# magicat777/Audio-Analyzer-OMEGA

Measured on AMD Instinct MI355X. Metric: audio frames/sec (multi-res FFT + LUFS + TruePeak) at 1/2/4/8 MI355X, higher is better.
Workload: dtype f32; 1 GPU; cfg2: 256 stereo frames x 16384 samples per GPU; MRFFT 16k/8k/4k/1k + combine(512) + K-weighted LUFS + 4x true peak + meter aggregates; channel_frames_per_gpu=512, frame_samples=16384, target_bins=512, parallelism=frames sharded over 1 GPU(s)

## Files before the change

audio-analyzer-omega_amd/csrc/capi.cpp:

```cpp
#include <hip/hip_runtime.h>

#include <algorithm>
#include <cmath>
#include <cstdarg>
#include <cstdio>
#include <cstdlib>
#include <cstring>
#include <exception>
#include <map>
#include <new>
#include <string>
#include <vector>

#include "../../include/omega.h"
#include "params.hpp"

namespace omega {
hipError_t launch_spectral(int W, const SpectralParams& p, hipStream_t s);
hipError_t launch_mrfft(const SpectralParams& p, hipStream_t s);
hipError_t launch_mrfft_range(const SpectralParams& p, int r0, int r1, hipStream_t s);
hipError_t launch_mrfft_independent(const SpectralParams& p, hipStream_t s);
hipError_t launch_truepeak(int W, const SpectralParams& p, hipStream_t s);
hipError_t launch_truepeak_rf(int W, const SpectralParams& p, hipStream_t s, int extra_lds = 0);
hipError_t launch_mrfft_rf(int n, const SpectralParams& p, int r, hipStream_t s);
// ... 167 lines not shown
  std::memcpy(P, An, sizeof P);
  double Pk[4] = {P[0], P[1], P[2], P[3]};
  for (int l = 0; l < 64; ++l) {
    for (int q = 0; q < 4; ++q) t.pw[l][q] = (float)Pk[q];
    mat2_mul(P, Pk, Pk);
  }
  return t;
}

}

struct omega_bands {
  omega_ctx* ctx;
  int op, n_bands, n_out, n_bins, n_valid;
  int32_t* d_starts;
  int32_t* d_ends;
  float* d_scale;
  float* d_bin_scale;
};

struct omega_ctx {
  omega_config cfg{};
  int device = 0;
  hipStream_t own = nullptr, stream = nullptr;
  hipStream_t cap = nullptr, fork[1] = {nullptr};
  std::vector<hipStream_t> spare;
  unsigned* d_probe = nullptr;
  unsigned probe_seq = 0;
  std::vector<hipStream_t> checked;
  bool queue_shared = false;
  hipEvent_t ev_fork = nullptr, ev_join[2] = {nullptr, nullptr};
  bool use_graph = false;
  int layout = 3;
  unsigned* d_kw_done = nullptr;
  unsigned kw_issued = 0;
  unsigned q_issued = 0;
  unsigned tp_issued = 0;
  unsigned prep_issued = 0;
  unsigned seg_issued = 0;
  unsigned lt_issued = 0;
  unsigned* tp_count_to = nullptr;
  bool side_meters = false;
  unsigned seg_par[2] = {0, 0};
  bool pipe = false;
  bool pend = false;
  MeterPrepParams pend_mq{};
  int pend_nq = 0, pend_par = 0;
  int stage_par = 0;
  unsigned* d_tail = nullptr;
  unsigned tail_issued = 0;
  unsigned long long* d_mirror = nullptr;
  unsigned mirror_gen = 0;
  int tail_ok = 0;
  unsigned* h_err = nullptr;
  unsigned* d_err = nullptr;
  int poll_limit = 1 << 22;
  float* d_lufs_scr = nullptr;
  int64_t lufs_scr_cap = 0;
  bool res_independent = false;
  hipEvent_t ev_kw = nullptr;
  struct GraphEntry {
    std::vector<uint64_t> key;
    hipGraph_t graph;
    hipGraphExec_t exec;
  };
  std::vector<GraphEntry> graphs;
  char err[512] = {};
  float2* d_tw[kMaxLog2] = {};

  float2* d_rot = nullptr;
  float* d_win[kMaxRes] = {};
  float* d_wgt[kMaxRes] = {};
  CombEnt* d_ent = nullptr;
  int ent_begin[kMaxRes] = {}, ent_end[kMaxRes] = {};
  int pair_lo[kMaxRes] = {}, pair_hi[kMaxRes] = {};
  int ent_jmax[kMaxRes] = {};
  std::map<std::pair<int, int>, BiquadTab*> kw_tabs;
  int rf_sizes = 1 << 14;
  std::map<std::pair<int, int>, float*> windows;
  std::map<int, float2*> rots;
  std::map<std::pair<int, int>, float4*> wgens;
  int* d_own_off = nullptr;
  int* d_own_rj = nullptr;
  float* d_own_frac = nullptr;
  std::map<int, std::pair<double*, std::pair<int, int>>> chroma_mats;
  double chroma_df = 0.0;
  struct ChromaTab {
    int n_bins = 0, lo = 0, hi = 0;
    double df = 0.0;
    float4* w4 = nullptr;
    float* w1 = nullptr;
    unsigned short* perm = nullptr;
    int* goff = nullptr;
    float* rec = nullptr;
  } ctab;
  int n_cu = 0;
  int drum_bins = 0, drum_cur = 0;
  float* d_dprev[2] = {};
  float* d_dhist[2] = {};
  int* d_dlen[2] = {};
  long long* d_dpos[2] = {};
  float* d_dflux = nullptr;
  PostParams post{};
  float* d_post_raw = nullptr;
  int64_t post_raw_cap = 0;
  double* d_vu_hist[2] = {};
// ... 58 lines not shown
  std::vector<void*> allocs;
};

namespace {

int fail(omega_ctx* c, int code, const char* fmt, ...) {
  char buf[512];
  va_list ap;
  va_start(ap, fmt);
  std::vsnprintf(buf, sizeof buf, fmt, ap);
  va_end(ap);
  if (c) {
    std::memcpy(c->err, buf, sizeof buf);
    c->zc_ok = false;
  }
  return code;
}

#define HIPC(ctx, x)                                                                           \
  do {                                                                                         \
    hipError_t e_ = (x);                                                                       \
    if (e_ != hipSuccess) return fail(ctx, OMEGA_EHIP, "%s: %s", #x, hipGetErrorString(e_)); \
  } while (0)

int guard_fail(omega_ctx* c) noexcept {
  try {
    throw;
  } catch (const std::bad_alloc&) {
    return fail(c, OMEGA_ENOMEM, "out of host memory");
  } catch (const std::exception& e) {
    return fail(c, OMEGA_EHIP, "internal error: %s", e.what());
  } catch (...) {
    return fail(c, OMEGA_EHIP, "internal error: unknown exception");
  }
}

template <class T>
int dalloc(omega_ctx* c, T** p, size_t count) {
  void* q = nullptr;
  const hipError_t e = hipMalloc(&q, std::max<size_t>(count, 1) * sizeof(T));
  if (e != hipSuccess) return fail(c, OMEGA_ENOMEM, "hipMalloc(%zu): %s", count * sizeof(T), hipGetErrorString(e));
  c->allocs.push_back(q);
  *p = static_cast<T*>(q);
  return 0;
}

template <class T>
int grow(omega_ctx* c, T** p, int64_t* cap, int64_t need) {
  if (need <= *cap) return 0;
  if (*p) {
    HIPC(c, hipStreamSynchronize(c->stream));
    for (hipStream_t f : c->fork)
      if (f) HIPC(c, hipStreamSynchronize(f));
    auto it = std::find(c->allocs.begin(), c->allocs.end(), static_cast<void*>(*p));
    if (it != c->allocs.end()) c->allocs.erase(it);
    (void)hipFree(*p);
    *p = nullptr;
    *cap = 0;
  }
  if (int e = dalloc(c, p, (size_t)need)) return e;
  *cap = need;
  return 0;
}

template <class T>
int upload(omega_ctx* c, T** p, const std::vector<T>& v) {
  int r = dalloc(c, p, v.size());
  if (r) return r;
  HIPC(c, hipMemcpy(*p, v.data(), v.size() * sizeof(T), hipMemcpyHostToDevice));
  return 0;
}

int stage_buf(omega_ctx* c, int i, size_t bytes, void** out) {
  if ((int)c->stage.size() <= i) c->stage.resize(i + 1);
  DevBuf& b = c->stage[i];
  if (b.n < bytes) {
    if (b.p) (void)hipFree(b.p);
    b.p = nullptr;
    b.n = 0;
    const hipError_t e = hipMalloc(&b.p, std::max<size_t>(bytes, 256));
    if (e != hipSuccess) return fail(c, OMEGA_ENOMEM, "staging hipMalloc(%zu): %s", bytes, hipGetErrorString(e));
    b.n = std::max<size_t>(bytes, 256);
  }
  *out = b.p;
  return 0;
}

int build_twiddles(omega_ctx* c) {
  for (int l = 1; l < kMaxLog2; ++l) {
    const int N = 1 << l;
    std::vector<float2> t(N);
    for (int m = 0; m < N; ++m) {
      const double a = 2.0 * kPi * (double)m / (double)N;
      t[m] = make_float2((float)std::cos(a), (float)-std::sin(a));
    }
    int r = upload(c, &c->d_tw[l], t);
    if (r) return r;
  }
  return 0;
}

int get_kw_tab(omega_ctx* c, int M, int L, BiquadTab** out) {
  const auto key = std::make_pair(M, L);
  auto it = c->kw_tabs.find(key);
  if (it != c->kw_tabs.end()) {
    *out = it->second;
    return 0;
  }
  const double fs = c->cfg.sample_rate;
  std::vector<BiquadTab> t = {make_biquad_tab(butter2_highpass(38.0, fs), L),
                              make_biquad_tab(butter2_highpass(1500.0, fs), L)};
  BiquadTab* d = nullptr;
  int r = upload(c, &d, t);
  if (r) return r;
  c->kw_tabs[key] = d;
  *out = d;
  return 0;
}
int get_kw_tab(omega_ctx* c, int M, BiquadTab** out) { return get_kw_tab(c, M, kw_chunk(M), out); }

int get_window(omega_ctx* c, int m, int kind, float** out) {
  auto key = std::make_pair(m, kind);
  auto it = c->windows.find(key);
  if (it != c->windows.end()) {
    *out = it->second;
    return 0;
  }
  float* d = nullptr;
  int r = upload(c, &d, make_window(m, kind));
  if (r) return r;
// ... 451 lines not shown
    p.n_t_in = c->d_nt[a];
    p.skeys_in = c->d_skeys[a];
    p.n_s_in = c->d_ns[a];
    p.t0_in = c->d_t0[a];
    p.hist_l_out = c->d_hist_l[b];
    p.hist_t_out = c->d_hist_t[b];
    p.n_l_out = c->d_nl[b];
    p.n_t_out = c->d_nt[b];
    p.skeys_out = c->d_skeys[b];
    p.n_s_out = c->d_ns[b];
    p.t0_out = c->d_t0[b];
    p.HL = c->HL;
    p.HT = c->HT;
    p.mom_len = c->cfg.momentary_len;
    p.short_len = c->cfg.short_len;
    p.int_len = c->cfg.integrated_len;
    p.peak_len = c->cfg.peak_len;
    p.poll_limit = c->poll_limit;
    p.err_word = c->d_err;
    p.gate = (float)c->cfg.gate_lufs;
    p.core = c->d_core[a];
    p.ext = c->d_ext[a];
    p.n_core = c->d_ncore[a];
    p.n_ext = c->d_next[a];
    p.gcount = c->d_gcount[a];
    p.gsum = c->d_gsum[a];
    p.out = out + f0 * C * OMEGA_N_METERS;
    p.parts = 3;
    p.seg_ctr = c->d_kw_done + 4;
    p.seg_pre_target = c->seg_par[a];
    p.seg_post_target = c->seg_par[b];
    v.push_back(p);
    c->cur = b;
  }
  return v;
}

int meters_enqueue(omega_ctx* c, const float* lufs, const float* tp, int64_t n_frames, double* out,
                   hipStream_t stream, hipEvent_t tp_ready, unsigned* wait_ctr = nullptr, unsigned wait_target = 0) {
  bool first = true;
  for (MeterPrepParams p : meter_chunks(c, lufs, tp, n_frames, out)) {
    if (first && wait_ctr) {
      p.wait_ctr = wait_ctr;
      p.wait_target = wait_target;
    }
    HIPC(c, launch_meter_prep(p, stream));
    if (tp_ready && first) HIPC(c, hipStreamWaitEvent(stream, tp_ready, 0));
    HIPC(c, launch_meter_query(p, stream));
    first = false;
  }
  return 0;
}

int flush_meters(omega_ctx* c) {
  if (!c->pend) return 0;
  HIPC(c, hipSetDevice(c->device));
  BatchPlan bp{};
  bp.q_begin = 0;
  bp.q_n = c->pend_nq;
  bp.seg_start[0] = bp.seg_start[1] = bp.multi_start = c->pend_nq;
  SpectralParams sp{};
  KWeightParams kp{};
  const hipError_t le = launch_batch(sp, kp, bp, c->pend_mq, c->pend_nq, c->stream);
  if (le != hipSuccess) return fail(c, OMEGA_EHIP, "meter segment launch: %s", hipGetErrorString(le));
  c->pend = false;
  c->seg_par[c->pend_par] = c->seg_issued + (unsigned)c->pend_nq;
  c->seg_issued += (unsigned)c->pend_nq;
  return 0;
}

bool batch_eligible(omega_ctx* c, const SpectralParams& sp, const KWeightParams& kp, int W, bool do_res, hipStream_t s,
                    int* mr) {
  *mr = -1;
  if (W != 16384 || (c->cap && s == c->cap)) return false;
  if ((kp.lufs_out || kp.weighted_out) && kp.mode != 0) return false;
  if (!do_res) return true;
  if (!c->res_independent) return false;
  for (int r = 0; r < sp.n_res; ++r) {
    if (!sp.comb_out && !sp.res[r].mag_out) continue;
    const int n = sp.res[r].n;
    if (n == 16384) {
      if (*mr >= 0 || !((sp.rf_sizes >> 14) & 1)) return false;
      *mr = r;
    } else if (n < 512 || n > 8192) {
      return false;
    }
  }
  return true;
}

int enqueue_batch(omega_ctx* c, SpectralParams sp, KWeightParams kp, int W, int64_t n_frames, const float* lufs,
                  const float* tp, double* meters, hipStream_t s, int mr, bool do_tp, bool do_kw, bool fold) {
  (void)W;
  const int64_t n = sp.n_cf;
  BatchPlan bp{};
  int seg[2][3], ns[2] = {0, 0};
  auto add = [&](int sg, int role, bool on) {
    if (on) seg[sg][ns[sg]++] = role;
  };
  add(0, 0, do_kw);
  add(0, 2, mr >= 0);
  add(1, 1, do_tp);
  const int64_t groups = (n + 7) / 8;
  int64_t end = 0;
  for (int sg = 0; sg < 2; ++sg) {
    bp.n_roles[sg] = ns[sg] ? ns[sg] : 1;
    for (int i = 0; i < 3; ++i) bp.roles[sg][i] = i < ns[sg] ? seg[sg][i] : 0;
    end += ns[sg] ? 8 * ns[sg] * groups : 0;
    if (end > 0x7FFFFFFF) return fail(c, OMEGA_EINVAL, "batch of %lld channel-frames too large", (long long)n);
    bp.seg_begin[sg + 1] = (int)end;
  }
  bp.mr_res = mr < 0 ? 0 : mr;
  int64_t nwg = 0;
  for (int r = 0; r < sp.n_res; ++r) {
    if (r == mr || (!sp.comb_out && !sp.res[r].mag_out)) continue;
    const int K = sp.res[r].n / 2;
    const int G = K / 16 < 64 ? 64 : K / 16;
    const int fpw = 512 / G;
    bp.multi.res[bp.multi.n_seg] = r;
    bp.multi.wg_begin[bp.multi.n_seg] = (int)nwg;
    ++bp.multi.n_seg;
    nwg += (n + fpw - 1) / fpw;
  }
  const bool in_grid = meters && do_tp && do_kw && n_frames > 0 && n_frames <= kChunkFrames;
  const int64_t n_mq = in_grid ? std::min<int64_t>((n + kBatchWaves - 1) / kBatchWaves, kMeterWgs) : 0;
  fold = fold && in_grid;
  const int64_t q_n = fold ? (c->pend ? c->pend_nq : 0) : n_mq;
  bp.pat = 1;
  bp.multi_n = (int)nwg;
  bp.seg_start[0] = 0;
  bp.seg_start[1] = bp.seg_begin[1];
  bp.multi_start = bp.seg_begin[2];
  const int64_t body_end = end + nwg;
  bp.q_begin = (int)body_end;
  bp.q_n = (int)q_n;
  if (fold) bp.q_begin = bp.multi_start;
  const int64_t grid = body_end + q_n;
  if (grid > 0x7FFFFFFF) return fail(c, OMEGA_EINVAL, "batch of %lld channel-frames too large", (long long)n);
  MeterPrepParams mq{};
  std::vector<MeterPrepParams> mc;
  if (in_grid) {
    const int a = c->cur;
    const unsigned seg_par_was = c->seg_par[a ^ 1];
    if (fold && c->pend) c->seg_par[c->pend_par] = c->seg_issued + (unsigned)c->pend_nq;
    const int cur_was = c->cur;
    mc = meter_chunks(c, lufs, tp, n_frames, meters);
    MeterPrepParams p = mc[0];
    p.q_done = c->d_kw_done + 3;
    const size_t mir_n = (size_t)kChunkFrames * c->cfg.n_channels;
    if (fold && !c->d_mirror) {
      HIPC(c, hipMalloc(&c->d_mirror, 2 * mir_n * sizeof(unsigned long long)));
      HIPC(c, hipMemset(c->d_mirror, 0, 2 * mir_n * sizeof(unsigned long long)));
    }
    const bool mirror = fold;
    const unsigned gen_was = c->mirror_gen;
    if (mirror) {
      c->mirror_gen = c->mirror_gen == 0xFFFFFFFFu ? 2u : c->mirror_gen + 1;
      kp.lufs_mirror = c->d_mirror + (c->mirror_gen & 1) * mir_n;
      kp.mirror_gen = c->mirror_gen;
      p.lufs_mirror = kp.lufs_mirror;
      p.mirror_gen = c->mirror_gen;
    } else {
      kp.kw_done = c->d_kw_done;
      c->kw_issued += (unsigned)n;
      p.wait_ctr = c->d_kw_done;
      p.wait_target = c->kw_issued;
    }
    if (fold && c->tail_ok == 0) {
      int ok = 0;
      HIPC(c, hipDeviceGetAttribute(&ok, hipDeviceAttributeCanUseStreamWaitValue, c->device));
      c->tail_ok = -1;
      if (ok && hipExtMallocWithFlags(reinterpret_cast<void**>(&c->d_tail), 8, hipMallocSignalMemory) == hipSuccess) {
        HIPC(c, hipMemset(c->d_tail, 0, 8));
        c->tail_issued = 0;
        c->tail_ok = 1;
      }
    }
    const bool tail = fold && c->tail_ok > 0;
    if (tail) bp.tail_ctr = c->d_tail;
    if (!fold) HIPC(c, launch_meter_prep(p, c->fork[0]));
    c->side_meters = true;
    mq = mc[0];
    mq.start_ctr = c->d_kw_done + 3;
    mq.start_target = c->prep_issued + (unsigned)p.C;
    if (!fold) {
      sp.tp_done = c->d_kw_done + 2;
      mq.join_ctr = c->d_kw_done + 2;
      mq.join_target = c->tp_issued + (unsigned)n;
    }
    const hipError_t le = launch_batch(sp, kp, bp, fold ? c->pend_mq : mq, (int)grid, s);
    if (le != hipSuccess) {
      if (!fold) {
        (void)hipMemcpy(c->d_kw_done, &c->kw_issued, sizeof(unsigned), hipMemcpyHostToDevice);
        c->prep_issued += (unsigned)p.C;
      } else {
        c->mirror_gen = gen_was;
        c->seg_par[a ^ 1] = seg_par_was;
        c->cur = cur_was;
      }
      return fail(c, OMEGA_EHIP, "batch launch: %s", hipGetErrorString(le));
    }
    if (!fold) c->tp_issued += (unsigned)n;
    if (tail) {
      HIPC(c, hipStreamWaitValue32(c->fork[0], c->d_tail, c->tail_issued + 1, hipStreamWaitValueGte, 0xFFFFFFFFu));
      ++c->tail_issued;
    }
    if (fold) HIPC(c, launch_meter_prep(p, c->fork[0]));
    c->side_meters = true;
    c->prep_issued += (unsigned)p.C;
    if (fold) {
      if (c->pend) c->seg_issued += (unsigned)c->pend_nq;
      c->pend = true;
      c->pend_mq = mq;
      c->pend_nq = (int)n_mq;
      c->pend_par = a;
    } else {
      c->seg_par[a] = c->seg_issued + (unsigned)n_mq;
      c->seg_issued += (unsigned)n_mq;
    }
    return 0;
  }
  if (meters) {
    mc = meter_chunks(c, lufs, tp, n_frames, meters);
    kp.kw_done = c->d_kw_done;
    c->kw_issued += (unsigned)n;
    for (size_t i = 0; i < mc.size(); ++i) {
      MeterPrepParams p = mc[i];
      if (i == 0) {
        p.wait_ctr = c->d_kw_done;
        p.wait_target = c->kw_issued;
      }
      HIPC(c, launch_meter_prep(p, c->fork[0]));
      c->side_meters = true;
      p.parts = 1;
      p.q_done = c->d_kw_done + 1;
      HIPC(c, launch_meter_query(p, c->fork[0]));
      c->side_meters = true;
      c->q_issued += (unsigned)(((p.n_frames + 3) / 4) * p.C);
    }
  }
  if (grid > 0) {
    const hipError_t le = launch_batch(sp, kp, bp, mq, (int)grid, s);
    if (le != hipSuccess) {
      if (meters) (void)hipMemcpy(c->d_kw_done, &c->kw_issued, sizeof(unsigned), hipMemcpyHostToDevice);
      return fail(c, OMEGA_EHIP, "batch launch: %s", hipGetErrorString(le));
    }
  }
  for (size_t i = 0; i < mc.size(); ++i) {
    MeterPrepParams p = mc[i];
    p.parts = 2;
    if (i + 1 == mc.size()) {
      p.join_ctr = c->d_kw_done + 1;
      p.join_target = c->q_issued;
    }
    HIPC(c, launch_meter_query(p, s));
  }
  return 0;
}

hipError_t create_side_stream(hipStream_t* st) { return hipStreamCreateWithFlags(st, hipStreamNonBlocking); }

constexpr int kProbePolls = 2048;
constexpr size_t kMaxSpare = 6;
int side_stream_check(omega_ctx* c, bool force = false) {
  if (!force && std::find(c->checked.begin(), c->checked.end(), c->stream) != c->checked.end()) return 0;
  if (!c->d_probe) {
    HIPC(c, hipMalloc(&c->d_probe, 2 * sizeof(unsigned)));
    HIPC(c, hipMemset(c->d_probe, 0, 2 * sizeof(unsigned)));
  }
  HIPC(c, hipStreamSynchronize(c->stream));
  HIPC(c, hipStreamSynchronize(c->fork[0]));
  for (int attempt = 0; attempt < 3; ++attempt) {
    const unsigned target = ++c->probe_seq;
    HIPC(c, launch_queue_probe(c->d_probe, target, kProbePolls, c->fork[0], c->stream));
    HIPC(c, hipStreamSynchronize(c->fork[0]));
    HIPC(c, hipStreamSynchronize(c->stream));
    unsigned r[2] = {0u, 0u};
    HIPC(c, hipMemcpy(r, c->d_probe, sizeof r, hipMemcpyDeviceToHost));
    if (r[1] == target) {
      c->queue_shared = false;
      c->checked.push_back(c->stream);
      return 0;
    }
    c->checked.clear();
    if (c->spare.size() >= kMaxSpare) {
      HIPC(c, hipStreamDestroy(c->spare.front()));
      c->spare.erase(c->spare.begin());
    }
    c->spare.push_back(c->fork[0]);
    c->fork[0] = nullptr;
    HIPC(c, create_side_stream(&c->fork[0]));
  }
  c->queue_shared = true;
  std::snprintf(c->err, sizeof c->err,
                "side stream: no hardware queue independent of the context's stream found after 3 attempts "
                "(more streams than GPU_MAX_HW_QUEUES?): batch-path device waits may run to their bound "
                "(OMEGA_POLL_LIMIT) and return OMEGA_EHIP");
  return 0;
}

int enqueue_frames(omega_ctx* c, SpectralParams sp, KWeightParams kp, int W, int64_t n_frames, const float* lufs,
                   const float* tp, double* meters, hipStream_t s, bool pipe = false, float* lufs_st = nullptr,
                   float* tp_st = nullptr) {
  const bool do_tp = sp.tp_out != nullptr, do_kw = kp.lufs_out || kp.weighted_out;
  const bool do_res = sp.comb_out != nullptr || sp.res[0].mag_out || sp.res[1].mag_out || sp.res[2].mag_out ||
                      sp.res[3].mag_out;
  int mr = -1;
  const bool batch = c->layout == 3 && batch_eligible(c, sp, kp, W, do_res, s, &mr);
  const bool fold = pipe && batch && meters && do_tp && do_kw && n_frames > 0 && n_frames <= kChunkFrames;
  if (c->pend && !fold)
    if (int e = flush_meters(c)) return e;
  if (fold && lufs_st && tp_st) {
    if (kp.lufs_out != lufs_st) kp.lufs_copy = kp.lufs_out;
    if (sp.tp_out != tp_st) sp.tp_copy = sp.tp_out;
    kp.lufs_out = lufs_st;
    sp.tp_out = tp_st;
    lufs = lufs_st;
    tp = tp_st;
  }
  if (batch) return enqueue_batch(c, sp, kp, W, n_frames, lufs, tp, meters, s, mr, do_tp, do_kw, fold);
  if (do_kw) HIPC(c, launch_kweight(W, kp, s));
  std::vector<MeterPrepParams> mc;
  if (meters) {
    mc = meter_chunks(c, lufs, tp, n_frames, meters);
    HIPC(c, hipEventRecord(c->ev_kw, s));
    HIPC(c, hipStreamWaitEvent(c->fork[0], c->ev_kw, 0));
    for (MeterPrepParams p : mc) {
      HIPC(c, launch_meter_prep(p, c->fork[0]));
      c->side_meters = true;
      p.parts = 1;
      HIPC(c, launch_meter_query(p, c->fork[0]));
      c->side_meters = true;
    }
    HIPC(c, hipEventRecord(c->ev_join[0], c->fork[0]));
  }
  if (do_res) HIPC(c, c->res_independent ? launch_mrfft_independent(sp, s) : launch_mrfft(sp, s));
  if (do_tp) HIPC(c, tp_launch(c, W, sp, s));
  for (MeterPrepParams p : mc) {
    p.parts = 2;
    HIPC(c, launch_meter_query(p, s));
  }
  if (meters) HIPC(c, hipStreamWaitEvent(s, c->ev_join[0], 0));
  return 0;
}

}

extern "C" {

const char* omega_version(void) { return "omega-mi355x 0.5 (gfx950, ABI 5)"; }

#ifdef OMEGA_STAMPS
int omega_dev_probe(omega_ctx* c, int which, const float* x, int64_t n_frames, float* comb, float* aux) {
  SpectralParams sp = spectral_params(c);
  const int W = c->cfg.frame_size;
  sp.x = x;
  sp.frame_stride = (int64_t)c->cfg.n_channels * W;
  sp.chan_stride = W;
  sp.n_cf = n_frames * c->cfg.n_channels;
  sp.comb_out = comb;
  (void)aux;
  for (int r = 0; r < kMaxRes; ++r) sp.res[r].mag_out = nullptr;
  hipError_t e = hipErrorInvalidValue;
  sp.tp_out = aux;
  float2* rot = nullptr;
  if (int r = get_rot(c, W, &rot)) return r;
  sp.rot = rot;
  if (which == 0) e = launch_mrfft_rf(16384, sp, 0, c->stream);
  if (which == 2) e = launch_truepeak_rf(16384, sp, c->stream);
  if (which == 3) e = launch_truepeak_rf(16384, sp, c->stream, 16 * 1024);
  return e == hipSuccess ? 0 : fail(c, OMEGA_EHIP, "probe %d: %s", which, hipGetErrorString(e));
// ... 902 lines not shown

int omega_post_reset(omega_ctx* c) try {
  if (!c) return OMEGA_EINVAL;
  if (!c->post.T) return 0;
  HIPC(c, hipSetDevice(c->device));
  HIPC(c, hipMemsetAsync(std::min(c->post.has_prev, c->post.has_prev_out), 0, 4 * sizeof(int), c->stream));
  HIPC(c, hipStreamSynchronize(c->stream));
  return 0;
} catch (...) {
  return guard_fail(c);
}

int omega_post_process(omega_ctx* c, const float* spectra, int64_t n_frames, int64_t stride, int32_t flags,
                       float bass_boost, float* spectrum_out, double* bands_out, int32_t* content_out) try {
  if (!c) return OMEGA_EINVAL;
  if (!c->post.T) return fail(c, OMEGA_EINVAL, "post process: omega_post_configure first");
  if (n_frames < 0 || stride < c->post.T || !spectra || !spectrum_out || (c->post.nb && !bands_out) ||
      n_frames > 0x7FFFFFFF)
    return fail(c, OMEGA_EINVAL, "post process: bad layout (n %lld, stride %lld, %d bins)", (long long)n_frames,
                (long long)stride, c->post.T);
  if (n_frames == 0) return 0;
  HIPC(c, hipSetDevice(c->device));
  PostParams p = c->post;
  p.in = spectra;
  p.n = n_frames;
  p.stride = stride;
  p.flags = flags;
  p.bass_boost = bass_boost;
  p.spec_out = spectrum_out;
  p.band_out = bands_out;
  p.content_out = content_out;
  const int64_t rows = n_frames + kEmaSpareRows, nch = (n_frames + 63) / 64;
  const int64_t pre_off = (rows * (c->post.nb + 1) + 1) / 2 * 2;
  if (c->post.nb) {
    if (int e = grow(c, &c->d_post_raw, &c->post_raw_cap, pre_off + 4 * nch * c->post.nb + 4)) return e;
  }
  p.band_raw = c->d_post_raw;
  p.frame64 = reinterpret_cast<int*>(c->d_post_raw + rows * c->post.nb);
  p.ema_pre = reinterpret_cast<double*>(c->d_post_raw + pre_off);
  p.ema_end = p.ema_pre + nch * c->post.nb;
  HIPC(c, launch_post(p, c->stream));
  if (c->post.nb) {
    std::swap(c->post.prev, c->post.prev_out);
    std::swap(c->post.has_prev, c->post.has_prev_out);
  }
  return 0;
} catch (...) {
  return guard_fail(c);
}

void omega_destroy(omega_ctx* c) try {
  if (!c) return;
  if (c->device >= 0) (void)hipSetDevice(c->device);
  if (c->pend && !flush_meters(c)) (void)hipStreamSynchronize(c->stream);
  if (c->own) (void)hipStreamSynchronize(c->own);
  if (c->fork[0]) (void)hipStreamSynchronize(c->fork[0]);
  for (void* p : c->allocs) (void)hipFree(p);
  for (auto& kv : c->chroma_mats) (void)hipFree(kv.second.first);
  for (void* q : {(void*)c->ctab.w4, (void*)c->ctab.w1, (void*)c->ctab.perm, (void*)c->ctab.goff,
                  (void*)c->ctab.rec})
    if (q) (void)hipFree(q);
  for (DevBuf& b : c->stage)
    if (b.p) (void)hipFree(b.p);
  for (DevBuf& b : c->pin)
    if (b.p) (void)hipHostFree(b.p);
  if (c->oarena.p) (void)hipFree(c->oarena.p);
  if (c->oarena_pin.p) (void)hipHostFree(c->oarena_pin.p);
  if (c->zc_pin.p) (void)hipHostFree(c->zc_pin.p);
  drop_graphs(c);
  if (c->h_err) (void)hipHostFree(c->h_err);
  if (c->d_tail) (void)hipFree(c->d_tail);
  if (c->d_mirror) (void)hipFree(c->d_mirror);
  for (hipStream_t st : {c->cap, c->fork[0]})
    if (st) (void)hipStreamDestroy(st);
  for (hipStream_t st : c->spare) (void)hipStreamDestroy(st);
  if (c->d_probe) (void)hipFree(c->d_probe);
  for (hipEvent_t ev : {c->ev_fork, c->ev_join[0], c->ev_join[1], c->ev_kw})
    if (ev) (void)hipEventDestroy(ev);
  if (c->own) (void)hipStreamDestroy(c->own);
  delete c;
} catch (...) {
}

const char* omega_last_error(const omega_ctx* c) { return c ? c->err : "null context"; }

int omega_set_stream(omega_ctx* c, void* s) try {
  if (!c) return OMEGA_EINVAL;
  const hipStream_t ns = static_cast<hipStream_t>(s);
  if (ns != c->stream) {
    if (c->pend) {
      HIPC(c, hipSetDevice(c->device));
      if (int e = flush_meters(c)) return e;
    }
    HIPC(c, hipSetDevice(c->device));
    HIPC(c, hipEventRecord(c->ev_fork, c->stream));
    HIPC(c, hipStreamWaitEvent(ns, c->ev_fork, 0));
    HIPC(c, hipStreamWaitEvent(c->fork[0], c->ev_fork, 0));
    c->stream = ns;
    if (int e = side_stream_check(c)) return e;
  }
  return 0;
} catch (...) {
  return guard_fail(c);
}

int omega_check_queues(omega_ctx* c, int* shared) try {
  if (!c) return OMEGA_EINVAL;
  HIPC(c, hipSetDevice(c->device));
  if (c->pend) {
    if (int e = flush_meters(c)) return e;
  }
  if (int e = side_stream_check(c, true)) return e;
  if (shared) *shared = c->queue_shared ? 1 : 0;
  return 0;
} catch (...) {
  return guard_fail(c);
}

void* omega_get_stream(const omega_ctx* c) { return c ? static_cast<void*>(c->stream) : nullptr; }

int omega_get_config(const omega_ctx* c, omega_config* cfg, int* device) {
  if (!c) return OMEGA_EINVAL;
  if (cfg) *cfg = c->cfg;
  if (device) *device = c->device;
  return 0;
}

int omega_set_graphs(omega_ctx* c, int enable) try {
  if (!c) return OMEGA_EINVAL;
  if (c->pend) {
    HIPC(c, hipSetDevice(c->device));
    if (int e = flush_meters(c)) return e;
  }
  c->use_graph = (enable & 1) != 0;
  c->layout = ((enable >> 1) & 3) ? 2 : 3;
  drop_graphs(c);
  return 0;
} catch (...) {
  return guard_fail(c);
}

int omega_synchronize(omega_ctx* c) try {
  if (!c) return OMEGA_EINVAL;
  if (c->pend) {
    HIPC(c, hipSetDevice(c->device));
    if (int e = flush_meters(c)) return e;
  }
  HIPC(c, hipStreamSynchronize(c->stream));
  return check_device_err(c);
} catch (...) {
  return guard_fail(c);
}

int omega_meter_reset(omega_ctx* c) try {
  if (!c) return OMEGA_EINVAL;
  if (int e = flush_meters(c)) return e;
  if (c->fork[0]) HIPC(c, hipStreamSynchronize(c->fork[0]));
  const int C = c->cfg.n_channels;
  for (int b = 0; b < 2; ++b) {
    HIPC(c, hipMemsetAsync(c->d_nl[b], 0, C * sizeof(int), c->stream));
    HIPC(c, hipMemsetAsync(c->d_nt[b], 0, C * sizeof(int), c->stream));
    HIPC(c, hipMemsetAsync(c->d_ns[b], 0, C * sizeof(int), c->stream));
    HIPC(c, hipMemsetAsync(c->d_t0[b], 0, C * sizeof(uint32_t), c->stream));
  }
  HIPC(c, hipStreamSynchronize(c->stream));
  return 0;
} catch (...) {
  return guard_fail(c);
}

int omega_process_frames(omega_ctx* c, const float* x, int64_t n_frames, int64_t frame_stride, int64_t channel_stride,
                         const omega_outputs* out, int mem) try {
  if (!c || !out) return OMEGA_EINVAL;
  if (!x || n_frames < 0) return fail(c, OMEGA_EINVAL, "null input or negative frame count");
  if (int e = check_device_err(c)) return e;
  if (n_frames == 0) return 0;
  const int C = c->cfg.n_channels, W = c->cfg.frame_size, T = c->cfg.target_bins;
  const int64_t ncf = n_frames * C;
  if ((frame_stride & 1) || (channel_stride & 1))
    return fail(c, OMEGA_EINVAL, "frame_stride and channel_stride must be even (8-byte aligned frames)");
  if (ncf > 0x7FFFFFFF) return fail(c, OMEGA_EINVAL, "too many channel-frames");
  HIPC(c, hipSetDevice(c->device));
  const bool pipe = c->pipe && mem == OMEGA_MEM_DEVICE && !c->use_graph;
  if (!pipe)
    if (int e = flush_meters(c)) return e;
  SpectralParams sp = spectral_params(c);
  sp.frame_stride = frame_stride;
  sp.chan_stride = channel_stride;
  sp.n_cf = ncf;
  std::vector<HostOut> outs;
  const float* dx = x;
  float* tp = out->true_peak_db;
  float* lufs = out->lufs_inst;
  double* meters = out->meters;
  float* comb = out->combined;
  float* weighted = out->weighted;
  float* mags[kMaxRes] = {};
// ... 20 lines not shown
  float* tp_st = nullptr;
  if (meters && (pipe || !lufs)) {
    e = stage_buf(c, 10 + sl, ncf * sizeof(float), reinterpret_cast<void**>(&lufs_st));
    if (e) return e;
    if (!lufs) lufs = lufs_st;
  }
  if (meters && (pipe || !tp)) {
    e = stage_buf(c, 11 + sl, ncf * sizeof(float), reinterpret_cast<void**>(&tp_st));
    if (e) return e;
    if (!tp) tp = tp_st;
  }
  sp.x = dx;
  sp.comb_out = comb;
  sp.tp_out = tp;
  for (int r = 0; r < c->cfg.n_res; ++r) sp.res[r].mag_out = mags[r];
  BiquadTab* tabs = nullptr;
  if (lufs || weighted) {
    e = get_kw_tab(c, W, &tabs);
    if (e) return e;
  }
  KWeightParams kp{dx, frame_stride, channel_stride, C, ncf, tabs, tabs ? tabs + 1 : nullptr, lufs, weighted, 0};
  if (mem == OMEGA_MEM_DEVICE && c->use_graph) {
    const std::vector<uint64_t> key = {(uint64_t)dx, (uint64_t)n_frames, (uint64_t)frame_stride,
                                       (uint64_t)channel_stride, (uint64_t)comb, (uint64_t)lufs, (uint64_t)tp,
                                       (uint64_t)meters, (uint64_t)weighted, (uint64_t)mags[0], (uint64_t)mags[1],
                                       (uint64_t)mags[2], (uint64_t)mags[3], (uint64_t)c->cur};
    hipGraphExec_t exec = nullptr;
    for (auto& g : c->graphs)
      if (g.key == key) exec = g.exec;
    if (!exec) {
      if (c->graphs.size() >= 16) {
        for (auto& g : c->graphs) {
          (void)hipGraphExecDestroy(g.exec);
          (void)hipGraphDestroy(g.graph);
        }
        c->graphs.clear();
      }
      const int cur0 = c->cur;
      if (!c->cap) HIPC(c, hipStreamCreateWithFlags(&c->cap, hipStreamNonBlocking));
      HIPC(c, hipStreamBeginCapture(c->cap, hipStreamCaptureModeThreadLocal));
      e = enqueue_frames(c, sp, kp, W, n_frames, lufs, tp, meters, c->cap);
      hipGraph_t graph = nullptr;
      const hipError_t ce = hipStreamEndCapture(c->cap, &graph);
      if (e) return e;
      if (ce != hipSuccess) return fail(c, OMEGA_EHIP, "graph capture: %s", hipGetErrorString(ce));
      HIPC(c, hipGraphInstantiate(&exec, graph, nullptr, nullptr, 0));
      c->graphs.push_back({key, graph, exec});
      c->cur = cur0;
    }
    HIPC(c, hipGraphLaunch(exec, c->stream));
    if (meters) c->cur ^= (int)(((n_frames + kChunkFrames - 1) / kChunkFrames) & 1);
    return 0;
  }
  e = enqueue_frames(c, sp, kp, W, n_frames, lufs, tp, meters, c->stream, pipe, lufs_st, tp_st);
  if (e) {
    if (pipe && meters) c->stage_par ^= 1;
    return e;
  }
  if (mem == OMEGA_MEM_HOST) return finish_host(c, outs);
  return 0;
} catch (...) {
  return guard_fail(c);
}

int omega_set_meter_pipelining(omega_ctx* c, int enable) try {
  if (!c) return OMEGA_EINVAL;
  if (!enable && c->pend) {
    HIPC(c, hipSetDevice(c->device));
    if (int e = flush_meters(c)) return e;
  }
  c->pipe = enable != 0;
  return 0;
} catch (...) {
  return guard_fail(c);
}

int omega_flush_meters(omega_ctx* c) try {
  if (!c) return OMEGA_EINVAL;
  if (!c->pend) return 0;
  HIPC(c, hipSetDevice(c->device));
  return flush_meters(c);
} catch (...) {
  return guard_fail(c);
}

int omega_process_stream(omega_ctx* c, const float* x, int64_t n_samples, int32_t hop, int64_t channel_stride,
                         const omega_outputs* out, int mem, int64_t* n_frames_out) try {
  if (!c) return OMEGA_EINVAL;
  if (n_frames_out) *n_frames_out = 0;
  if (hop < 1 || n_samples < 0) return fail(c, OMEGA_EINVAL, "hop must be >= 1 and n_samples >= 0");
  const int W = c->cfg.frame_size;
  const int64_t nf = n_samples < W ? 0 : (n_samples - W) / hop + 1;
  if (n_frames_out) *n_frames_out = nf;
  return omega_process_frames(c, x, nf, hop, channel_stride, out, mem);
} catch (...) {
  return guard_fail(c);
}

int omega_combine(omega_ctx* c, const float* const* mags, int64_t n_cf, float* out, int mem) try {
  if (!c || !mags || !out) return OMEGA_EINVAL;
  if (n_cf <= 0) return n_cf == 0 ? 0 : fail(c, OMEGA_EINVAL, "negative count");
  HIPC(c, hipSetDevice(c->device));
  const int T = c->cfg.target_bins;
  CombineParams p{};
  std::vector<HostOut> outs;
  float* dout = out;
  int e = 0;
  for (int r = 0; r < c->cfg.n_res; ++r) {
    p.nbins[r] = c->cfg.res[r].fft_size / 2 + 1;
    p.cw[r] = (float)c->cfg.res[r].weight;
    if (!mags[r]) continue;
    if (mem == OMEGA_MEM_HOST) {
      const void* d = nullptr;
      e = stage_in(c, 20 + r, mags[r], (size_t)n_cf * p.nbins[r] * sizeof(float), &d);
      if (e) return e;
      p.mag[r] = static_cast<const float*>(d);
    } else {
      p.mag[r] = mags[r];
    }
  }
  if (mem == OMEGA_MEM_HOST) {
    e = stage_out(c, 24, out, (size_t)n_cf * T, outs, &dout);
    if (e) return e;
  }
  p.n_cf = n_cf;
  p.T = T;
  p.own_off = c->d_own_off;
  p.own_rj = c->d_own_rj;
  p.own_frac = c->d_own_frac;
  p.out = dout;
  HIPC(c, launch_combine(p, c->stream));
  if (mem == OMEGA_MEM_HOST) return finish_host(c, outs);
// ... 680 lines not shown
```

audio-analyzer-omega_amd/omega_gpu/engine.py:

```python
from __future__ import annotations

import ctypes as C
from dataclasses import dataclass
from typing import Dict, Optional, Sequence, Tuple

import numpy as np

from . import _lib as L


@dataclass(frozen=True)
class Resolution:

    freq_range: Tuple[float, float]
    fft_size: int
    hop_size: int
    weight: float
    window: str = "blackman"


DEFAULT_RESOLUTIONS = (
    Resolution((20, 200), 4096, 1024, 1.5),
    Resolution((200, 1000), 2048, 512, 1.2),
    Resolution((1000, 5000), 1024, 256, 1.0),
# ... 110 lines not shown

    def _alloc(self, like, shape, dtype):
        if _is_torch(like):
            import torch
            tdt = {np.float32: torch.float32, np.float64: torch.float64}[dtype]
            return torch.empty(shape, dtype=tdt, device=like.device)
        return np.empty(shape, dtype=dtype)

    def process_stream(self, x, n_samples: int, hop: int, channel_stride: int = 0, **kw) -> Dict:
        n_frames = 0 if n_samples < self.W else (n_samples - self.W) // hop + 1
        return self.process_frames(x, n_frames, hop, channel_stride, _stream=(n_samples, hop), **kw)

    def process_frames(self, x, n_frames: int, frame_stride: int, channel_stride: int, *, combined=True,
                       lufs=True, true_peak=True, meters=False, mags=False, weighted=False,
                       out: Optional[Dict] = None, _stream=None) -> Dict:
        dev = _is_torch(x)
        if not dev:
            x = np.ascontiguousarray(x, dtype=np.float32)
        ncf = n_frames * self.C
        o = dict(out or {})
        if combined and "combined" not in o:
            o["combined"] = self._alloc(x, (ncf, self.T), np.float32)
        if lufs and "lufs_inst" not in o:
            o["lufs_inst"] = self._alloc(x, (ncf,), np.float32)
        if true_peak and "true_peak_db" not in o:
            o["true_peak_db"] = self._alloc(x, (ncf,), np.float32)
        if meters and "meters" not in o:
            o["meters"] = self._alloc(x, (ncf, L.N_METERS), np.float64)
        if weighted and "weighted" not in o:
            o["weighted"] = self._alloc(x, (ncf, self.W), np.float32)
        if mags:
            sel = range(len(self.resolutions)) if mags is True else mags
            for r in sel:
                o.setdefault(f"mag{r}", self._alloc(x, (ncf, self.resolutions[r].fft_size // 2 + 1), np.float32))
        outs = L.Outputs()
        outs.combined = _ptr(o.get("combined"))
        outs.lufs_inst = _ptr(o.get("lufs_inst"))
        outs.true_peak_db = _ptr(o.get("true_peak_db"))
        outs.meters = _ptr(o.get("meters"))
        outs.weighted = _ptr(o.get("weighted"))
        for r in range(len(self.resolutions)):
            outs.mag[r] = _ptr(o.get(f"mag{r}"))
        if dev:
            self._bind_stream(x)
        mem = L.MEM_DEVICE if dev else L.MEM_HOST
        if _stream is not None:
            got = C.c_int64(0)
            self._check(L.lib().omega_process_stream(self._ctx, _ptr(x), int(_stream[0]), int(_stream[1]),
                                                     int(channel_stride), C.byref(outs), mem, C.byref(got)))
            assert got.value == n_frames
        else:
            self._check(L.lib().omega_process_frames(self._ctx, _ptr(x), int(n_frames), int(frame_stride),
                                                     int(channel_stride), C.byref(outs), mem))
        self._held = o if (self._pipe and dev and meters) else None
        return o

    def combine(self, mags: Dict[int, np.ndarray], n_cf: int = 1) -> np.ndarray:
        arrs = {i: np.ascontiguousarray(m, dtype=np.float32) for i, m in mags.items()}
        ptrs = (C.c_void_p * L.MAX_RES)()
        for i in range(L.MAX_RES):
            ptrs[i] = arrs[i].ctypes.data if i in arrs else None
        out = np.empty((n_cf, self.T), np.float32)
        self._check(L.lib().omega_combine(self._ctx, ptrs, int(n_cf), out.ctypes.data, L.MEM_HOST))
        return out

    def true_peak(self, x: np.ndarray, oversampling: int = 4) -> np.ndarray:
        x = np.ascontiguousarray(np.atleast_2d(x), dtype=np.float32)
        out = np.empty(x.shape[0], np.float32)
        self._check(L.lib().omega_true_peak_os(self._ctx, x.ctypes.data, x.shape[0], x.shape[1], int(oversampling),
                                               out.ctypes.data, L.MEM_HOST))
        return out

    def weighting(self, x: np.ndarray, mode: str = "K", weighted: bool = True):
        x = np.ascontiguousarray(np.atleast_2d(x), dtype=np.float32)
        w = np.empty_like(x) if weighted else None
        li = np.empty(x.shape[0], np.float32)
        self._check(L.lib().omega_weighting(self._ctx, x.ctypes.data, x.shape[0], x.shape[1], L.WEIGHT[mode],
                                            w.ctypes.data if w is not None else None, li.ctypes.data, L.MEM_HOST))
        return w, li

    def k_weighting(self, x: np.ndarray, weighted: bool = True):
        return self.weighting(x, "K", weighted)

    def k_weighting_scan(self, x: np.ndarray, weighted: bool = True):
        x = np.ascontiguousarray(np.atleast_2d(x), dtype=np.float32)
        w = np.empty_like(x) if weighted else None
        li = np.empty(x.shape[0], np.float32)
        self._check(L.lib().omega_k_weighting(self._ctx, x.ctypes.data, x.shape[0], x.shape[1],
                                              w.ctypes.data if w is not None else None, li.ctypes.data, L.MEM_HOST))
        return w, li

    def load_meter_history(self, lufs_inst, tp_db):
        if _is_torch(lufs_inst):
            import torch
            li, tp = lufs_inst.contiguous(), tp_db.contiguous()
            if li.dtype != torch.float32 or tp.dtype != torch.float32:
                raise ValueError("load_meter_history: float32 rows")
            if li.numel():
                self._bind_stream(li)
            mem = L.MEM_DEVICE
        else:
            li = np.ascontiguousarray(lufs_inst, dtype=np.float32)
            tp = np.ascontiguousarray(tp_db, dtype=np.float32)
            mem = L.MEM_HOST
        n_l, n_t = li.shape[0] if li.ndim else 0, tp.shape[0] if tp.ndim else 0
        if li.ndim != 2 or li.shape[1] != self.C or (n_t and (tp.ndim != 2 or tp.shape[1] != self.C)):
            raise ValueError(f"load_meter_history: [n, {self.C}] rows")
# ... 119 lines not shown
```

Measured before the change: 8.440 million channel-frames/s.

## Overlap consecutive pipelined batch calls on two alternating batch streams

Adds two dedicated batch streams that pipelined, meter-folded batch calls alternate between. Each call waits on the caller's stream and the previous tail counter, then records a done event, so consecutive calls can overlap on the GPU instead of serialising on one stream. A host-side overlap check on input and output buffer spans forces a join when calls alias memory. The cost is extra events, stream waits and a queue-independence probe, and the path only runs when meter pipelining is enabled and the batch path with fold applies.

Result: faster. 8.761 million channel-frames/s, median of 6 (+3.8%).

```diff
diff --git a/audio-analyzer-omega_amd/csrc/capi.cpp b/audio-analyzer-omega_amd/csrc/capi.cpp
--- a/audio-analyzer-omega_amd/csrc/capi.cpp
+++ b/audio-analyzer-omega_amd/csrc/capi.cpp
@@ -243,6 +243,13 @@
   unsigned long long* d_mirror = nullptr;
   unsigned mirror_gen = 0;
   int tail_ok = 0;
+  hipStream_t bs[2] = {nullptr, nullptr};
+  hipEvent_t ev_in = nullptr, ev_done[2] = {nullptr, nullptr};
+  unsigned bs_idx = 0;
+  int last_bs = 0;
+  bool unjoined = false;
+  bool bs_shared = false;
+  std::vector<std::pair<const char*, size_t>> prev_span;
   unsigned* h_err = nullptr;
   unsigned* d_err = nullptr;
   int poll_limit = 1 << 22;
@@ -407,6 +414,8 @@
     HIPC(c, hipStreamSynchronize(c->stream));
     for (hipStream_t f : c->fork)
       if (f) HIPC(c, hipStreamSynchronize(f));
+    for (hipStream_t f : c->bs)
+      if (f) HIPC(c, hipStreamSynchronize(f));
     auto it = std::find(c->allocs.begin(), c->allocs.end(), static_cast<void*>(*p));
     if (it != c->allocs.end()) c->allocs.erase(it);
     (void)hipFree(*p);
@@ -430,7 +439,11 @@
   if ((int)c->stage.size() <= i) c->stage.resize(i + 1);
   DevBuf& b = c->stage[i];
   if (b.n < bytes) {
-    if (b.p) (void)hipFree(b.p);
+    if (b.p) {
+      for (hipStream_t f : c->bs)
+        if (f) HIPC(c, hipStreamSynchronize(f));
+      (void)hipFree(b.p);
+    }
     b.p = nullptr;
     b.n = 0;
     const hipError_t e = hipMalloc(&b.p, std::max<size_t>(bytes, 256));
@@ -988,7 +1001,18 @@
   return 0;
 }
 
-int flush_meters(omega_ctx* c) {
+int join_batches(omega_ctx* c) {
+  if (!c->unjoined) return 0;
+  HIPC(c, hipSetDevice(c->device));
+  HIPC(c, hipStreamWaitEvent(c->stream, c->ev_done[c->last_bs], 0));
+  c->unjoined = false;
+  c->prev_span.clear();
+  return 0;
+}
+
+int flush_meters(omega_ctx* c, hipStream_t on = nullptr) {
+  if (!on)
+    if (int e = join_batches(c)) return e;
   if (!c->pend) return 0;
   HIPC(c, hipSetDevice(c->device));
   BatchPlan bp{};
@@ -997,11 +1021,24 @@
   bp.seg_start[0] = bp.seg_start[1] = bp.multi_start = c->pend_nq;
   SpectralParams sp{};
   KWeightParams kp{};
-  const hipError_t le = launch_batch(sp, kp, bp, c->pend_mq, c->pend_nq, c->stream);
+  const hipError_t le = launch_batch(sp, kp, bp, c->pend_mq, c->pend_nq, on ? on : c->stream);
   if (le != hipSuccess) return fail(c, OMEGA_EHIP, "meter segment launch: %s", hipGetErrorString(le));
   c->pend = false;
   c->seg_par[c->pend_par] = c->seg_issued + (unsigned)c->pend_nq;
   c->seg_issued += (unsigned)c->pend_nq;
+  return 0;
+}
+
+int tail_init(omega_ctx* c) {
+  if (c->tail_ok != 0) return 0;
+  int ok = 0;
+  HIPC(c, hipDeviceGetAttribute(&ok, hipDeviceAttributeCanUseStreamWaitValue, c->device));
+  c->tail_ok = -1;
+  if (ok && hipExtMallocWithFlags(reinterpret_cast<void**>(&c->d_tail), 8, hipMallocSignalMemory) == hipSuccess) {
+    HIPC(c, hipMemset(c->d_tail, 0, 8));
+    c->tail_issued = 0;
+    c->tail_ok = 1;
+  }
   return 0;
 }
 
@@ -1102,16 +1139,8 @@
       p.wait_ctr = c->d_kw_done;
       p.wait_target = c->kw_issued;
     }
-    if (fold && c->tail_ok == 0) {
-      int ok = 0;
-      HIPC(c, hipDeviceGetAttribute(&ok, hipDeviceAttributeCanUseStreamWaitValue, c->device));
-      c->tail_ok = -1;
-      if (ok && hipExtMallocWithFlags(reinterpret_cast<void**>(&c->d_tail), 8, hipMallocSignalMemory) == hipSuccess) {
-        HIPC(c, hipMemset(c->d_tail, 0, 8));
-        c->tail_issued = 0;
-        c->tail_ok = 1;
-      }
-    }
+    if (fold)
+      if (int e = tail_init(c)) return e;
     const bool tail = fold && c->tail_ok > 0;
     if (tail) bp.tail_ctr = c->d_tail;
     if (!fold) HIPC(c, launch_meter_prep(p, c->fork[0]));
@@ -1198,6 +1227,60 @@
 
 constexpr int kProbePolls = 2048;
 constexpr size_t kMaxSpare = 6;
+int replace_side_stream(omega_ctx* c, hipStream_t* st) {
+  hipStream_t fresh = nullptr;
+  HIPC(c, create_side_stream(&fresh));
+  c->spare.push_back(*st);
+  *st = fresh;
+  if (c->spare.size() > kMaxSpare) {
+    HIPC(c, hipStreamDestroy(c->spare.front()));
+    c->spare.erase(c->spare.begin());
+  }
+  return 0;
+}
+
+int probe_pair(omega_ctx* c, hipStream_t waiter, hipStream_t setter, bool* ind) {
+  const unsigned target = ++c->probe_seq;
+  HIPC(c, launch_queue_probe(c->d_probe, target, kProbePolls, waiter, setter));
+  HIPC(c, hipStreamSynchronize(waiter));
+  HIPC(c, hipStreamSynchronize(setter));
+  unsigned r[2] = {0u, 0u};
+  HIPC(c, hipMemcpy(r, c->d_probe, sizeof r, hipMemcpyDeviceToHost));
+  *ind = r[1] == target;
+  return 0;
+}
+
+int batch_stream_check(omega_ctx* c) {
+  c->bs_shared = false;
+  if (!c->bs[0]) return 0;
+  if (!c->d_probe) {
+    HIPC(c, hipMalloc(&c->d_probe, 2 * sizeof(unsigned)));
+    HIPC(c, hipMemset(c->d_probe, 0, 2 * sizeof(unsigned)));
+  }
+  HIPC(c, hipStreamSynchronize(c->stream));
+  HIPC(c, hipStreamSynchronize(c->fork[0]));
+  for (int k = 0; k < 2; ++k) {
+    HIPC(c, hipStreamSynchronize(c->bs[k]));
+    bool ind = false;
+    for (int attempt = 0;; ++attempt) {
+      if (int e = probe_pair(c, c->fork[0], c->bs[k], &ind)) return e;
+      if (ind)
+        if (int e = probe_pair(c, c->bs[k], c->stream, &ind)) return e;
+      if (ind && k == 1)
+        if (int e = probe_pair(c, c->bs[0], c->bs[1], &ind)) return e;
+      if (ind || attempt == 3) break;
+      if (int e = replace_side_stream(c, &c->bs[k])) return e;
+    }
+    if (!ind) c->bs_shared = true;
+  }
+  if (c->bs_shared && !c->queue_shared)
+    std::snprintf(c->err, sizeof c->err,
+                  "batch streams: no hardware queues independent of the context's stream, the side stream and "
+                  "each other found after 3 attempts (more streams than GPU_MAX_HW_QUEUES?): consecutive "
+                  "pipelined batch calls serialise instead of overlapping");
+  return 0;
+}
+
 int side_stream_check(omega_ctx* c, bool force = false) {
   if (!force && std::find(c->checked.begin(), c->checked.end(), c->stream) != c->checked.end()) return 0;
   if (!c->d_probe) {
@@ -1216,35 +1299,34 @@
     if (r[1] == target) {
       c->queue_shared = false;
       c->checked.push_back(c->stream);
-      return 0;
+      return batch_stream_check(c);
     }
     c->checked.clear();
-    if (c->spare.size() >= kMaxSpare) {
-      HIPC(c, hipStreamDestroy(c->spare.front()));
-      c->spare.erase(c->spare.begin());
-    }
-    c->spare.push_back(c->fork[0]);
-    c->fork[0] = nullptr;
-    HIPC(c, create_side_stream(&c->fork[0]));
+    if (int e = replace_side_stream(c, &c->fork[0])) return e;
   }
   c->queue_shared = true;
+  if (int e = batch_stream_check(c)) return e;
   std::snprintf(c->err, sizeof c->err,
                 "side stream: no hardware queue independent of the context's stream found after 3 attempts "
                 "(more streams than GPU_MAX_HW_QUEUES?): batch-path device waits may run to their bound "
-                "(OMEGA_POLL_LIMIT) and return OMEGA_EHIP");
+                "(OMEGA_POLL_LIMIT) and return OMEGA_EHIP%s",
+                c->bs_shared ? "; the batch streams share queues too: pipelined batch calls serialise" : "");
   return 0;
 }
 
 int enqueue_frames(omega_ctx* c, SpectralParams sp, KWeightParams kp, int W, int64_t n_frames, const float* lufs,
                    const float* tp, double* meters, hipStream_t s, bool pipe = false, float* lufs_st = nullptr,
-                   float* tp_st = nullptr) {
+                   float* tp_st = nullptr, bool serial = false) {
   const bool do_tp = sp.tp_out != nullptr, do_kw = kp.lufs_out || kp.weighted_out;
   const bool do_res = sp.comb_out != nullptr || sp.res[0].mag_out || sp.res[1].mag_out || sp.res[2].mag_out ||
                       sp.res[3].mag_out;
   int mr = -1;
   const bool batch = c->layout == 3 && batch_eligible(c, sp, kp, W, do_res, s, &mr);
   const bool fold = pipe && batch && meters && do_tp && do_kw && n_frames > 0 && n_frames <= kChunkFrames;
-  if (c->pend && !fold)
+  if (fold && c->bs[0])
+    if (int e = tail_init(c)) return e;
+  const bool ovl = fold && c->bs[0] && c->tail_ok > 0;
+  if ((c->pend && (!fold || ovl)) || (c->unjoined && !ovl))
     if (int e = flush_meters(c)) return e;
   if (fold && lufs_st && tp_st) {
     if (kp.lufs_out != lufs_st) kp.lufs_copy = kp.lufs_out;
@@ -1253,6 +1335,36 @@
     sp.tp_out = tp_st;
     lufs = lufs_st;
     tp = tp_st;
+  }
+  if (ovl) {
+    const int k = (int)(c->bs_idx & 1);
+    hipStream_t b = c->bs[k];
+    if (serial)
+      if (int e = join_batches(c)) return e;
+    HIPC(c, hipEventRecord(c->ev_in, s));
+    HIPC(c, hipStreamWaitEvent(b, c->ev_in, 0));
+    if (c->tail_issued)
+      HIPC(c, hipStreamWaitValue32(b, c->d_tail, c->tail_issued, hipStreamWaitValueGte, 0xFFFFFFFFu));
+    const int err = [&]() -> int {
+      if (int e = enqueue_batch(c, sp, kp, W, n_frames, lufs, tp, meters, b, mr, do_tp, do_kw, true)) return e;
+      if (c->unjoined) HIPC(c, hipStreamWaitEvent(b, c->ev_done[k ^ 1], 0));
+      if (int e = flush_meters(c, b)) return e;
+      HIPC(c, hipEventRecord(c->ev_done[k], b));
+      if (c->unjoined) HIPC(c, hipStreamWaitEvent(s, c->ev_done[k ^ 1], 0));
+      return 0;
+    }();
+    if (err) {
+      (void)hipEventRecord(c->ev_done[k], b);
+      if (c->unjoined) (void)hipStreamWaitEvent(s, c->ev_done[k ^ 1], 0);
+      (void)hipStreamWaitEvent(s, c->ev_done[k], 0);
+      c->unjoined = false;
+      c->prev_span.clear();
+      return err;
+    }
+    c->unjoined = true;
+    c->last_bs = k;
+    ++c->bs_idx;
+    return 0;
   }
   if (batch) return enqueue_batch(c, sp, kp, W, n_frames, lufs, tp, meters, s, mr, do_tp, do_kw, fold);
   if (do_kw) HIPC(c, launch_kweight(W, kp, s));
@@ -2261,7 +2373,9 @@
 void omega_destroy(omega_ctx* c) try {
   if (!c) return;
   if (c->device >= 0) (void)hipSetDevice(c->device);
-  if (c->pend && !flush_meters(c)) (void)hipStreamSynchronize(c->stream);
+  if ((c->pend || c->unjoined) && !flush_meters(c)) (void)hipStreamSynchronize(c->stream);
+  for (hipStream_t st : c->bs)
+    if (st) (void)hipStreamSynchronize(st);
   if (c->own) (void)hipStreamSynchronize(c->own);
   if (c->fork[0]) (void)hipStreamSynchronize(c->fork[0]);
   for (void* p : c->allocs) (void)hipFree(p);
@@ -2280,11 +2394,11 @@
   if (c->h_err) (void)hipHostFree(c->h_err);
   if (c->d_tail) (void)hipFree(c->d_tail);
   if (c->d_mirror) (void)hipFree(c->d_mirror);
-  for (hipStream_t st : {c->cap, c->fork[0]})
+  for (hipStream_t st : {c->cap, c->fork[0], c->bs[0], c->bs[1]})
     if (st) (void)hipStreamDestroy(st);
   for (hipStream_t st : c->spare) (void)hipStreamDestroy(st);
   if (c->d_probe) (void)hipFree(c->d_probe);
-  for (hipEvent_t ev : {c->ev_fork, c->ev_join[0], c->ev_join[1], c->ev_kw})
+  for (hipEvent_t ev : {c->ev_fork, c->ev_join[0], c->ev_join[1], c->ev_kw, c->ev_in, c->ev_done[0], c->ev_done[1]})
     if (ev) (void)hipEventDestroy(ev);
   if (c->own) (void)hipStreamDestroy(c->own);
   delete c;
@@ -2297,7 +2411,7 @@
   if (!c) return OMEGA_EINVAL;
   const hipStream_t ns = static_cast<hipStream_t>(s);
   if (ns != c->stream) {
-    if (c->pend) {
+    if (c->pend || c->unjoined) {
       HIPC(c, hipSetDevice(c->device));
       if (int e = flush_meters(c)) return e;
     }
@@ -2316,7 +2430,7 @@
 int omega_check_queues(omega_ctx* c, int* shared) try {
   if (!c) return OMEGA_EINVAL;
   HIPC(c, hipSetDevice(c->device));
-  if (c->pend) {
+  if (c->pend || c->unjoined) {
     if (int e = flush_meters(c)) return e;
   }
   if (int e = side_stream_check(c, true)) return e;
@@ -2337,7 +2451,7 @@
 
 int omega_set_graphs(omega_ctx* c, int enable) try {
   if (!c) return OMEGA_EINVAL;
-  if (c->pend) {
+  if (c->pend || c->unjoined) {
     HIPC(c, hipSetDevice(c->device));
     if (int e = flush_meters(c)) return e;
   }
@@ -2351,7 +2465,7 @@
 
 int omega_synchronize(omega_ctx* c) try {
   if (!c) return OMEGA_EINVAL;
-  if (c->pend) {
+  if (c->pend || c->unjoined) {
     HIPC(c, hipSetDevice(c->device));
     if (int e = flush_meters(c)) return e;
   }
@@ -2478,11 +2592,31 @@
     if (meters) c->cur ^= (int)(((n_frames + kChunkFrames - 1) / kChunkFrames) & 1);
     return 0;
   }
-  e = enqueue_frames(c, sp, kp, W, n_frames, lufs, tp, meters, c->stream, pipe, lufs_st, tp_st);
+  std::vector<std::pair<const char*, size_t>> span_now;
+  bool serial = false;
+  if (pipe) {
+    auto add = [&](const void* p, size_t bytes) {
+      if (p) span_now.emplace_back(static_cast<const char*>(p), bytes);
+    };
+    span_now.emplace_back(reinterpret_cast<const char*>(x), span * sizeof(float));
+    add(comb, (size_t)ncf * T * sizeof(float));
+    add(out->lufs_inst, (size_t)ncf * sizeof(float));
+    add(out->true_peak_db, (size_t)ncf * sizeof(float));
+    add(meters, (size_t)ncf * OMEGA_N_METERS * sizeof(double));
+    add(weighted, (size_t)ncf * W * sizeof(float));
+    for (int r = 0; r < c->cfg.n_res; ++r) add(mags[r], (size_t)ncf * (c->cfg.res[r].fft_size / 2 + 1) * sizeof(float));
+    if (c->unjoined)
+      for (size_t i = 0; i < span_now.size() && !serial; ++i)
+        for (size_t j = 0; j < c->prev_span.size() && !serial; ++j)
+          serial = (i || j) && span_now[i].first < c->prev_span[j].first + c->prev_span[j].second &&
+                   c->prev_span[j].first < span_now[i].first + span_now[i].second;
+  }
+  e = enqueue_frames(c, sp, kp, W, n_frames, lufs, tp, meters, c->stream, pipe, lufs_st, tp_st, serial);
   if (e) {
     if (pipe && meters) c->stage_par ^= 1;
     return e;
   }
+  if (c->unjoined) c->prev_span.swap(span_now);
   if (mem == OMEGA_MEM_HOST) return finish_host(c, outs);
   return 0;
 } catch (...) {
@@ -2491,11 +2625,20 @@
 
 int omega_set_meter_pipelining(omega_ctx* c, int enable) try {
   if (!c) return OMEGA_EINVAL;
-  if (!enable && c->pend) {
+  if (!enable && (c->pend || c->unjoined)) {
     HIPC(c, hipSetDevice(c->device));
     if (int e = flush_meters(c)) return e;
   }
   c->pipe = enable != 0;
+  if (c->pipe && !c->bs[0]) {
+    HIPC(c, hipSetDevice(c->device));
+    for (int k = 0; k < 2; ++k) {
+      HIPC(c, create_side_stream(&c->bs[k]));
+      HIPC(c, hipEventCreateWithFlags(&c->ev_done[k], hipEventDisableTiming));
+    }
+    HIPC(c, hipEventCreateWithFlags(&c->ev_in, hipEventDisableTiming));
+    if (int e = batch_stream_check(c)) return e;
+  }
   return 0;
 } catch (...) {
   return guard_fail(c);
@@ -2503,7 +2646,7 @@
 
 int omega_flush_meters(omega_ctx* c) try {
   if (!c) return OMEGA_EINVAL;
-  if (!c->pend) return 0;
+  if (!c->pend && !c->unjoined) return 0;
   HIPC(c, hipSetDevice(c->device));
   return flush_meters(c);
 } catch (...) {
diff --git a/audio-analyzer-omega_amd/omega_gpu/engine.py b/audio-analyzer-omega_amd/omega_gpu/engine.py
--- a/audio-analyzer-omega_amd/omega_gpu/engine.py
+++ b/audio-analyzer-omega_amd/omega_gpu/engine.py
@@ -186,7 +186,7 @@
         else:
             self._check(L.lib().omega_process_frames(self._ctx, _ptr(x), int(n_frames), int(frame_stride),
                                                      int(channel_stride), C.byref(outs), mem))
-        self._held = o if (self._pipe and dev and meters) else None
+        self._held = (o, x) if (self._pipe and dev and meters) else None
         return o
 
     def combine(self, mags: Dict[int, np.ndarray], n_cf: int = 1) -> np.ndarray:
```
